# HUBioDataLab/DrugGEN

Measured on AMD Instinct MI355X. Metric: molecules/sec GAN step (G+D fwd+bwd), N=45 graphs, higher is better.
Workload: dtype f32

## Files before the change

druggen_amd/csrc/row_gemm.hip:

```cpp
#include "common.h"
#include "f16_scale.h"
#include "lane_reduce.h"
#include "row_gemm.h"
#include "row_gemm_n384.h"
#include "row_gemm_k384.h"
#include "traversal.h"

#include <cstring>
#include <type_traits>

namespace dg {
namespace {

typedef float f32x16 __attribute__((ext_vector_type(16)));

constexpr int kTR = 64;

struct Epilogue {
    const float* bias = nullptr;
    float* y_alt[2] = {nullptr, nullptr};
    const float* residual = nullptr;
    const float* gamma = nullptr;
    const float* beta = nullptr;
    float* mean = nullptr;
    float* rstd = nullptr;
    float* pre = nullptr;
    float eps = 0.f;
    int relu = 0;
    const float* lnb_pre = nullptr;
    float* lnb_part = nullptr;
    const float* lna_pre = nullptr;
    float* lna_dz = nullptr;
    const float* bias_alt[2] = {nullptr, nullptr};
    int reverse = 0;
};

__device__ __forceinline__ float half_sum(float x) { return half_wave_total_readlane(x, threadIdx.x & 32); }

constexpr int kH3Pitch = 272;
constexpr int kH3Plane = kTR * kH3Pitch;
constexpr int kH3Rs = 2 * kH3Plane;
constexpr int kH3Buf = kH3Rs + kTR * 4;
constexpr int kH3Lds = 2 * kH3Buf;
static_assert(kH3Rs >= kTR * 128 * 4, "the fp32 exchange tile must not reach the row scales");


template <int PFN, int STRIDE>
__device__ __forceinline__ void split_write_h3(const float4 (&set)[PFN], char* pl, int pt) {
    constexpr int G = PFN > 8 ? 2 : 4;
    static_assert(PFN % G == 0 && STRIDE % 32 == 0, "whole groups, whole rows");
    char* const prow = pl + (pt >> 5) * kH3Pitch + (pt & 31) * 8;
    char* const prs = pl + kH3Rs + (pt >> 5) * 4;
#pragma unroll
    for (int g0 = 0; g0 < PFN; g0 += G) {
        unsigned m[G];
#pragma unroll
        for (int j = 0; j < G; ++j) {
            const float4& v = set[g0 + j];
            float t, u;
            asm("v_max3_f32 %0, |%1|, |%2|, |%3|" : "=v"(t) : "v"(v.x), "v"(v.y), "v"(v.z));
            asm("v_max_f32_e64 %0, |%1|, %2" : "=v"(u) : "v"(v.w), "v"(t));
            m[j] = __float_as_uint(u);
        }
#pragma unroll
        for (int j = 0; j < G; ++j) m[j] = umax_dpp<0xB1>(m[j]);
#pragma unroll
        for (int j = 0; j < G; ++j) m[j] = umax_dpp<0x4E>(m[j]);
#pragma unroll
        for (int j = 0; j < G; ++j) m[j] = umax_dpp<0x141>(m[j]);
#pragma unroll
        for (int j = 0; j < G; ++j) m[j] = umax_dpp<0x140>(m[j]);
        float sc[G];
#pragma unroll
        for (int j = 0; j < G; ++j) {
            const auto r = __builtin_amdgcn_permlane16_swap(m[j], m[j], false, false);
            const unsigned x = r[0] > r[1] ? r[0] : r[1];
            const unsigned e = max(x >> 23, 15u);
            m[j] = e;
            sc[j] = scale_of(e);
        }
        f32x2 xa[G], xb[G];
        f16x2 ha[G], hb[G];
#pragma unroll
        for (int j = 0; j < G; ++j) {
            const float4& v = set[g0 + j];
            xa[j] = f32x2{v.x, v.y} * sc[j];
            xb[j] = f32x2{v.z, v.w} * sc[j];
        }
#pragma unroll
        for (int j = 0; j < G; ++j) {
            ha[j] = __builtin_convertvector(xa[j], f16x2);
            hb[j] = __builtin_convertvector(xb[j], f16x2);
        }
#pragma unroll
        for (int j = 0; j < G; ++j) {
            xa[j] -= __builtin_convertvector(ha[j], f32x2);
            xb[j] -= __builtin_convertvector(hb[j], f32x2);
        }
#pragma unroll
        for (int j = 0; j < G; ++j) {
            const f16x2 la = __builtin_convertvector(xa[j], f16x2), lb = __builtin_convertvector(xb[j], f16x2);
            const u32x2 h = {__builtin_bit_cast(unsigned, ha[j]), __builtin_bit_cast(unsigned, hb[j])};
            const u32x2 l = {__builtin_bit_cast(unsigned, la), __builtin_bit_cast(unsigned, lb)};
            *reinterpret_cast<u32x2*>(prow + 0 * kH3Plane + (STRIDE / 32) * (g0 + j) * kH3Pitch) = h;
            *reinterpret_cast<u32x2*>(prow + 1 * kH3Plane + (STRIDE / 32) * (g0 + j) * kH3Pitch) = l;
        }
        if ((pt & 31) == 0) {
#pragma unroll
            for (int j = 0; j < G; ++j)
                *reinterpret_cast<float*>(prs + (STRIDE / 32) * (g0 + j) * 4) = inv_scale_of(m[j]);
        }
    }
}

__device__ __forceinline__ void pack_weight_h3_block(const float* __restrict__ w, const float* __restrict__ w1,
                                                     const float* __restrict__ w2, f16x8* __restrict__ p, int rows, int cols,
                                                     int mode, int n_tiles, int t, int kcb, int kchunks) {
    __shared__ unsigned part[16][32];
    const int k_steps = 8 * kchunks;
    const int lane = threadIdx.x & 63, ks = threadIdx.x >> 6;
    const int c = lane & 31, n = 32 * t + c;
    const int n_out = mode == 0 ? rows : cols, kdim = mode == 0 ? cols : rows;
    auto at = [&](int k) -> float {
        if (n >= n_out || k >= kdim) return 0.f;
        int r = mode == 0 ? n : k;
        const int c = mode == 0 ? k : n;
        const float* ws = w;
        if (w1) {
            ws = r < 128 ? w : (r < 256 ? w1 : w2);
            r &= 127;
        }
        return ws[static_cast<size_t>(r) * cols + c];
    };
    float v[8];
    unsigned mx = 0;
    for (int kc = 0; kc < kchunks; ++kc)
#pragma unroll
        for (int j = 0; j < 8; ++j) {
            const float x = at(kc * 128 + ks * 16 + 8 * (lane >> 5) + j);
            if (kc == kcb) v[j] = x;
            mx = max(mx, __float_as_uint(x) & 0x7FFFFFFFu);
        }
    part[2 * ks + (lane >> 5)][c] = mx;
    __syncthreads();
#pragma unroll
    for (int i = 0; i < 16; ++i) mx = max(mx, part[i][c]);
    const unsigned e = scale_exponent(__uint_as_float(mx));
    const float sc = scale_of(e);
    f16x8 hi, lo;
#pragma unroll
    for (int j = 0; j < 8; ++j) {
        const float xs = v[j] * sc;
        hi[j] = static_cast<_Float16>(xs);
        lo[j] = static_cast<_Float16>(xs - static_cast<float>(hi[j]));
    }
    const size_t slot = static_cast<size_t>(t) * k_steps + 8 * kcb + ks;
    p[(slot * 2 + 0) * 64 + lane] = hi;
    p[(slot * 2 + 1) * 64 + lane] = lo;
    if (kcb == 0 && ks == 0 && lane < 32)
        reinterpret_cast<float*>(p + static_cast<size_t>(n_tiles) * k_steps * 2 * 64)[n] = inv_scale_of(e);
}
__global__ __launch_bounds__(512) void pack_weight_h3_kernel(const float* __restrict__ w, const float* __restrict__ w1,
                                                             const float* __restrict__ w2, f16x8* __restrict__ p, int rows,
                                                             int cols, int mode, int n_tiles) {
    pack_weight_h3_block(w, w1, w2, p, rows, cols, mode, n_tiles, blockIdx.x, blockIdx.y, gridDim.y);
}
__global__ __launch_bounds__(512) void pack_weight_h3_batch_kernel(const long long* __restrict__ table) {
    const long long* e = table + 7 * static_cast<size_t>(blockIdx.z);
    const float* w = reinterpret_cast<const float*>(e[0]);
    f16x8* p = reinterpret_cast<f16x8*>(e[1]);
    const int rows = static_cast<int>(e[2]), cols = static_cast<int>(e[3]), mode = static_cast<int>(e[4]);
    const int n_out = mode == 0 ? rows : cols, k = mode == 0 ? cols : rows;
    const int nt = (n_out + 31) / 32, kc = (k + 127) / 128;
    if (static_cast<int>(blockIdx.x) >= nt || static_cast<int>(blockIdx.y) >= kc) return;
    pack_weight_h3_block(w, reinterpret_cast<const float*>(e[5]), reinterpret_cast<const float*>(e[6]), p, rows, cols, mode,
                         nt, blockIdx.x, blockIdx.y, kc);
}

template <int NG, bool EXCH, bool LNB = false, bool LNA = false>
__global__ __launch_bounds__(512, 2) void row_gemm_h3_kernel(const float* __restrict__ a, const f16x8* __restrict__ packed,
                                                             float* __restrict__ y, int64_t R, Epilogue ep) {
    constexpr int NC = 4, NM = 8 - NC, PFN = 2048 / (64 * NM);
    constexpr int K = 128, KS = 8;
    static_assert(!LNB || (EXCH && NG == 1), "LayerNorm-backward epilogue: 128 -> 128 exchange kernel");
    static_assert(!LNA || (!EXCH && !LNB && NG == 1), "LayerNorm-backward prologue: plain 128 -> 128 kernel");
    static_assert(NG == 1 || (NG == 3 && !EXCH && !LNB && !LNA), "three outputs: direct epilogue, one column group per Linear");
    constexpr int DEPTH = LNA ? 2 : 3;
    extern __shared__ __attribute__((aligned(16))) char smem_raw[];
    char* lds = smem_raw;
    float* xb = reinterpret_cast<float*>(smem_raw + kH3Lds);
    const int lane = threadIdx.x & 63;
    const int w = __builtin_amdgcn_readfirstlane(threadIdx.x >> 6);
    const int half = lane >> 5, col = lane & 31;
    const int64_t tiles = (R + kTR - 1) / kTR;
    if (static_cast<int64_t>(blockIdx.x) >= tiles) return;
    const int64_t my_tiles = (tiles - blockIdx.x + gridDim.x - 1) / gridDim.x;
    const int64_t nchunks = my_tiles;
    const int rot = static_cast<int>(blockIdx.x % 3);
    const int64_t padded = (nchunks + DEPTH - 1) / DEPTH * DEPTH;
    auto tile_at = [&](int64_t ti) {
        const int64_t t = blockIdx.x + ti * gridDim.x;
        if constexpr (LNB || LNA || NG == 3) return t;
        else return ep.reverse ? tiles - 1 - t : t;
    };

    if (w >= NC) {
        const int pt = threadIdx.x - 64 * NC;
        if constexpr (LNA) {
            constexpr int K_ = 128;
            float4 dyr[2][PFN], prr[PFN];
            float st;
            const float4 gam = ld4(ep.gamma + (pt & 31) * 4);
            float4 dgam = f4(0.f), dbet = f4(0.f);
            const unsigned voff0 = static_cast<unsigned>(pt >> 5) * (K_ * 4) + static_cast<unsigned>(pt & 31) * 16;
            auto offsets = [&](int64_t chunk, int64_t& r0, unsigned& lim) {
                r0 = tile_at(chunk) * kTR;
                const int64_t last = R - 1 - r0;
                lim = last >= kTR - 1 ? 0xFFFFFFFFu
                                      : static_cast<unsigned>(last) * (K_ * 4) + static_cast<unsigned>(pt & 31) * 16;
            };
            auto fetch_dy = [&](auto s_tag, int64_t chunk) {
                constexpr int s = decltype(s_tag)::value;
                if (chunk > nchunks - 1) chunk = nchunks - 1;
                int64_t r0;
                unsigned lim;
                offsets(chunk, r0, lim);
                const char* ba = reinterpret_cast<const char*>(a) + r0 * (K_ * 4);
#pragma unroll
                for (int i = 0; i < PFN; ++i) {
                    unsigned off = voff0 + i * (2 * NM * K_ * 4);
                    off = off < lim ? off : lim;
                    dyr[s][i] = ld4(reinterpret_cast<const float*>(ba + off));
                }
            };
            auto fetch_pre = [&](int64_t chunk) {
                if (chunk > nchunks - 1) chunk = nchunks - 1;
                int64_t r0;
                unsigned lim;
                offsets(chunk, r0, lim);
                const char* bp = reinterpret_cast<const char*>(ep.lna_pre) + r0 * (K_ * 4);
#pragma unroll
                for (int i = 0; i < PFN; ++i) {
                    unsigned off = voff0 + i * (2 * NM * K_ * 4);
                    off = off < lim ? off : lim;
                    prr[i] = ld4(reinterpret_cast<const float*>(bp + off));
                }
                int64_t row = r0 + (pt >> 5) + 8 * (pt & 7);
                if (row > R - 1) row = R - 1;
                st = (pt & 8) ? ep.rstd[row] : ep.mean[row];
            };
            auto write2 = [&](auto s_tag, int64_t chunk) {
                constexpr int s = decltype(s_tag)::value;
                const float live = chunk < nchunks ? 1.f : 0.f;
                const int buf = static_cast<int>(chunk & 1);
                if (chunk > nchunks - 1) chunk = nchunks - 1;
                int64_t r0;
                unsigned lim;
                offsets(chunk, r0, lim);
                char* bz = reinterpret_cast<char*>(ep.lna_dz) + r0 * (K_ * 4);
                const int64_t last = R - 1 - r0;
                const unsigned lastu = static_cast<unsigned>(last < kTR - 1 ? last : kTR - 1);
                unsigned rowt = static_cast<unsigned>(pt) >> 5;
                asm volatile("" : "+v"(rowt));
                const int sti = __float_as_int(st);
#pragma unroll
                for (int i0 = 0; i0 < PFN; i0 += 4) {
                    float4 dzs[4];
#pragma unroll
                    for (int i = i0; i < i0 + 4; ++i) {
                        const int mu0 = __builtin_amdgcn_readlane(sti, i), mu1 = __builtin_amdgcn_readlane(sti, 32 + i);
                        const int rs0 = __builtin_amdgcn_readlane(sti, 8 + i), rs1 = __builtin_amdgcn_readlane(sti, 40 + i);
                        const float mu = __int_as_float(half ? mu1 : mu0), rs = __int_as_float(half ? rs1 : rs0);
                        const float4 v = dyr[s][i];
                        const float4 xh = rs * (prr[i] - f4(mu));
                        const float4 u = v * gam;
                        const float c1 = half_sum((u.x + u.y) + (u.z + u.w)) * (1.0f / 128.0f);
                        const float c2 = half_sum((u.x * xh.x + u.y * xh.y) + (u.z * xh.z + u.w * xh.w)) * (1.0f / 128.0f);
                        const float4 dz = rs * (u - f4(c1) - c2 * xh);
                        const float ok = rowt + 8u * i <= lastu ? live : 0.f;
                        const float4 vm = ok * v;
                        dgam = fma4(vm, xh, dgam);
                        dbet += vm;
                        dzs[i - i0] = dz;
                        unsigned off = voff0 + i * (2 * NM * K_ * 4);
                        off = off < lim ? off : lim;
                        st4(reinterpret_cast<float*>(bz + off), dz);
                    }
                    __builtin_amdgcn_sched_barrier(0);
                    split_write_h3<4, 64 * NM>(dzs, lds + buf * kH3Buf, pt + i0 * (64 * NM));
                    __builtin_amdgcn_sched_barrier(0);
                }
                fetch_pre(chunk + 1);
            };
            constexpr std::integral_constant<int, 0> S0{};
            constexpr std::integral_constant<int, 1> S1{};
            fetch_dy(S0, 0);
            fetch_pre(0);
            fetch_dy(S1, 1);
            write2(S0, 0);
            fetch_dy(S0, 2);
            __syncthreads();
            for (int64_t c = 0; c < padded; c += 2) {
                write2(S1, c + 1);
                fetch_dy(S1, c + 3);
                __syncthreads();
                write2(S0, c + 2);
                fetch_dy(S0, c + 4);
                __syncthreads();
            }
            float* pp = ep.lnb_part + (static_cast<size_t>(blockIdx.x) * 8 + 2 * (w - NC) + half) * 256 + (pt & 31) * 4;
            st4(pp, dgam);
            st4(pp + 128, dbet);
            return;
        }
        float4 pf[3][PFN];
        const unsigned voff0 = static_cast<unsigned>(pt >> 5) * (K * 4) + static_cast<unsigned>(pt & 31) * 16;
        auto fetch = [&](float4 (&set)[PFN], int64_t chunk) {
            if (chunk > nchunks - 1) chunk = nchunks - 1;
            const int64_t r0 = tile_at(chunk) * kTR;
            const char* base = reinterpret_cast<const char*>(a) + r0 * (K * 4);
            const int64_t last = R - 1 - r0;
            const unsigned lim = last >= kTR - 1 ? 0xFFFFFFFFu
                                                 : static_cast<unsigned>(last) * (K * 4) + static_cast<unsigned>(pt & 31) * 16;
#pragma unroll
            for (int i = 0; i < PFN; ++i) {
                unsigned off = voff0 + i * (2 * NM * K * 4);
                off = off < lim ? off : lim;
                set[i] = ld4(reinterpret_cast<const float*>(base + off));
            }
        };
        auto write = [&](const float4 (&set)[PFN], int64_t chunk) {
            split_write_h3<PFN, 64 * NM>(set, lds + (chunk & 1) * kH3Buf, pt);
        };
        auto end_of_iteration = [&](int64_t c) {
            if (EXCH && c < nchunks) {
                __syncthreads();
                __syncthreads();
            }
            __syncthreads();
        };
        fetch(pf[0], 0);
        fetch(pf[1], 1);
        fetch(pf[2], 2);
        write(pf[0], 0);
        fetch(pf[0], 3);
        __syncthreads();
        for (int64_t c = 0; c < padded; c += 3) {
            write(pf[1], c + 1);
            fetch(pf[1], c + 4);
            end_of_iteration(c);
            write(pf[2], c + 2);
            fetch(pf[2], c + 5);
            end_of_iteration(c + 1);
            write(pf[0], c + 3);
            fetch(pf[0], c + 6);
            end_of_iteration(c + 2);
        }
        return;
    }

    f16x8 bset[2][2][4];
    auto slab_of = [&](int g) { return 4 * g + w; };
    auto load_b = [&](f16x8 (&bfr)[2][4], int g, int h) {
        const f16x8* wp = packed + static_cast<size_t>(slab_of(g)) * KS * 2 * 64 + lane;
#pragma unroll
        for (int ks = 0; ks < 4; ++ks)
#pragma unroll
            for (int p = 0; p < 2; ++p) bfr[p][ks] = wp[((4 * h + ks) * 2 + p) * 64];
    };
    const float* inv_cs = reinterpret_cast<const float*>(packed + static_cast<size_t>(4 * NG) * KS * 2 * 64);
    float bias_g[NG], cs_g[NG];
#pragma unroll
    for (int g = 0; g < NG; ++g) {
        const int n = 32 * slab_of(g) + col;
        if (NG == 3) {
            const float* bp = n < 128 ? ep.bias : ep.bias_alt[(n >> 7) - 1];
            bias_g[g] = bp ? bp[n & 127] : 0.f;
        } else {
            bias_g[g] = ep.bias ? ep.bias[n] : 0.f;
        }
        cs_g[g] = inv_cs[n];
    }
    float4 res[8];
    float4 lpre[LNB ? 4 : 1];
    float4 dgam = f4(0.f), dbet = f4(0.f);
    f32x16 acc[2];
    auto unit = [&](int64_t ti, int pos_g) {
        const int g = NG > 1 ? (pos_g + rot) % NG : 0;
        const int64_t chunk = ti;
        const int64_t tix = tile_at(ti);
        const int64_t r0 = tix * kTR;
        if (NG > 1) load_b(bset[1], g, 1);
#pragma unroll
        for (int m = 0; m < 2; ++m)
#pragma unroll
            for (int i = 0; i < 16; ++i) acc[m][i] = 0.f;
        unsigned colv = static_cast<unsigned>(col), halfv = static_cast<unsigned>(half);
        if (EXCH) asm volatile("" : "+v"(colv), "+v"(halfv));
        const unsigned lastr = static_cast<unsigned>(R - 1 - r0 < kTR - 1 ? R - 1 - r0 : kTR - 1);
        auto row_off = [&](int it) {
            unsigned rr = static_cast<unsigned>(w * 16 + it * 2) + halfv;
            rr = rr < lastr ? rr : lastr;
            return rr * 512u + colv * 16u;
        };
        if (EXCH && ep.residual) {
            const char* rbase = reinterpret_cast<const char*>(ep.residual) + r0 * 512;
#pragma unroll
            for (int it = 0; it < 8; ++it) res[it] = ld4(reinterpret_cast<const float*>(rbase + row_off(it)));
        }
        const char* pl = lds + (chunk & 1) * kH3Buf;
        f16x8 af[2][2][2];
        auto frags = [&](int ks, f16x8 (&dst)[2][2]) {
#pragma unroll
            for (int m = 0; m < 2; ++m)
#pragma unroll
                for (int p = 0; p < 2; ++p)
                    dst[m][p] = *reinterpret_cast<const f16x8*>(pl + p * kH3Plane + (32 * m + col) * kH3Pitch +
                                                                (ks * 16 + 8 * half) * 2);
        };
        auto row_scales = [&](float4 (&rs)[4], int m, float cs) {
            const float* rsp = reinterpret_cast<const float*>(pl + kH3Rs);
#pragma unroll
            for (int q = 0; q < 4; ++q) rs[q] = cs * ld4(rsp + 32 * m + 8 * q + 4 * half);
        };
        frags(0, af[0]);
#pragma unroll
        for (int ks = 0; ks < 8; ++ks) {
            if (ks + 1 < 8) frags(ks + 1, af[(ks + 1) & 1]);
            if (NG > 1 && ks == 4) {
                const int un = (pos_g + 1) % NG;
                load_b(bset[0], (un + rot) % NG, 0);
            }
            const f16x8(&f)[2][2] = af[ks & 1];
            const f16x8(&bfr)[2][4] = bset[ks >> 2];
            constexpr int TA[3] = {1, 0, 0}, TB[3] = {0, 1, 0};
#pragma unroll
            for (int t = 0; t < 3; ++t)
#pragma unroll
                for (int m = 0; m < 2; ++m)
                    acc[m] = __builtin_amdgcn_mfma_f32_32x32x16_f16(f[m][TA[t]], bfr[TB[t]][ks & 3], acc[m], 0, 0, 0);
        }
        if (!EXCH) {
            const bool full = r0 + kTR <= R;
            const float bias = bias_g[g];
            float* yb = y;
            if constexpr (NG == 3) {
                if (g > 0) yb = ep.y_alt[g - 1];
            }
#pragma unroll
            for (int m = 0; m < 2; ++m) {
                float out[16];
                float4 rs[4];
                row_scales(rs, m, cs_g[g]);
#pragma unroll
                for (int reg = 0; reg < 16; ++reg) {
                    float v = fmaf(acc[m][reg], comp(rs[reg >> 2], reg & 3), bias);
                    if (ep.relu) v = fmaxf(v, 0.f);
                    out[reg] = v;
                }
                float* xw = xb + w * (32 * 32);
#pragma unroll
                for (int reg = 0; reg < 16; ++reg) xw[((reg & 3) + 8 * (reg >> 2) + 4 * half) * 32 + col] = out[reg];
                __builtin_amdgcn_wave_barrier();
                float4 rowv[4];
#pragma unroll
                for (int i = 0; i < 4; ++i) rowv[i] = ld4(xw + (8 * i + (lane >> 3)) * 32 + 4 * (lane & 7));
                __builtin_amdgcn_wave_barrier();
                float* yr = yb + (r0 + 32 * m + (lane >> 3)) * 128 + 32 * w + 4 * (lane & 7);
                if (full) {
#pragma unroll
                    for (int i = 0; i < 4; ++i) st4(yr + static_cast<size_t>(8 * i) * 128, rowv[i]);
                } else {
#pragma unroll
                    for (int i = 0; i < 4; ++i)
                        if (r0 + 32 * m + 8 * i + (lane >> 3) < R) st4(yr + static_cast<size_t>(8 * i) * 128, rowv[i]);
                }
            }
        }
        if (EXCH) {
            float* ex = reinterpret_cast<float*>(lds + (chunk & 1) * kH3Buf);
            const float bias = bias_g[0];
            float4 rs[2][4];
            row_scales(rs[0], 0, cs_g[0]);
            row_scales(rs[1], 1, cs_g[0]);
            if (LNB) {
                const char* pbase = reinterpret_cast<const char*>(ep.lnb_pre) + r0 * 512;
#pragma unroll
                for (int it = 0; it < 4; ++it) lpre[LNB ? it : 0] = ld4(reinterpret_cast<const float*>(pbase + row_off(it)));
            }
            __syncthreads();
#pragma unroll
            for (int m = 0; m < 2; ++m)
#pragma unroll
                for (int reg = 0; reg < 16; ++reg) {
                    const int rr = 32 * m + (reg & 3) + 8 * (reg >> 2) + 4 * half;
                    float v = fmaf(acc[m][reg], comp(rs[m][reg >> 2], reg & 3), bias);
                    if (ep.relu) v = fmaxf(v, 0.f);
                    ex[rr * 128 + 32 * w + col] = v;
                }
            __syncthreads();
            auto finish_rows_lnb = [&](auto check_tag) {
                constexpr bool CHECK = decltype(check_tag)::value;
                float* yrow = reinterpret_cast<float*>(reinterpret_cast<char*>(y + r0 * 128) + ((w * 16 + halfv) * 512u + colv * 16u));
                const float4 gam = ld4(reinterpret_cast<const float*>(reinterpret_cast<const char*>(ep.gamma) + colv * 16u));
#pragma unroll
                for (int hg = 0; hg < 2; ++hg) {
                    float4 pn[4];
                    if (hg == 0) {
                        const char* pbase = reinterpret_cast<const char*>(ep.lnb_pre) + r0 * 512;
#pragma unroll
                        for (int j = 0; j < 4; ++j) pn[j] = ld4(reinterpret_cast<const float*>(pbase + row_off(4 + j)));
                    }
                    float mu4[4], rs4[4];
#pragma unroll
                    for (int j = 0; j < 4; ++j) {
                        unsigned rr = static_cast<unsigned>(w * 16 + (4 * hg + j) * 2) + halfv;
                        rr = rr < lastr ? rr : lastr;
                        mu4[j] = ep.mean[r0 + rr];
                        rs4[j] = ep.rstd[r0 + rr];
                    }
                    float4 yv[4];
#pragma unroll
                    for (int j = 0; j < 4; ++j) {
                        const int it = 4 * hg + j, rr = w * 16 + it * 2 + half;
                        float4 v = ld4(reinterpret_cast<const float*>(reinterpret_cast<const char*>(ex) + ((w * 16 + it * 2 + halfv) * 512u + colv * 16u)));
                        if (ep.residual) v += res[it];
                        if (CHECK && static_cast<unsigned>(w * 16 + it * 2) + halfv > lastr) v = f4(0.f);
                        const float4 xh = rs4[j] * (lpre[LNB ? j : 0] - f4(mu4[j]));
                        const float4 u = v * gam;
                        const float c1 = half_sum((u.x + u.y) + (u.z + u.w)) * (1.0f / 128.0f);
                        const float c2 = half_sum((u.x * xh.x + u.y * xh.y) + (u.z * xh.z + u.w * xh.w)) * (1.0f / 128.0f);
                        yv[j] = rs4[j] * (u - f4(c1) - c2 * xh);
                        dgam = fma4(v, xh, dgam);
                        dbet += v;
                    }
#pragma unroll
                    for (int j = 0; j < 4; ++j) {
                        const int it = 4 * hg + j, rr = w * 16 + it * 2 + half;
                        if (!CHECK || static_cast<unsigned>(w * 16 + it * 2) + halfv <= lastr) st4(yrow + it * 256, yv[j]);
                        if (hg == 0) lpre[LNB ? j : 0] = pn[j];
                    }
                }
            };
            auto finish_rows = [&](auto check_tag) {
                constexpr bool CHECK = decltype(check_tag)::value;
                float* yrow = y + (r0 + w * 16 + half) * 128 + col * 4;
                float* prow = ep.pre ? ep.pre + (r0 + w * 16 + half) * 128 + col * 4 : nullptr;
                float4 gam = f4(0.f), bet = f4(0.f);
                if (ep.gamma) {
                    gam = ld4(ep.gamma + col * 4);
                    bet = ld4(ep.beta + col * 4);
                }
                float4 yv[8], pv[8];
                float mu8[8], rs8[8];
#pragma unroll
                for (int it = 0; it < 8; ++it) {
                    const int rr = w * 16 + it * 2 + half;
                    float4 v = ld4(ex + rr * 128 + col * 4);
                    if (ep.residual) v += res[it];
                    pv[it] = v;
                    if (ep.gamma) {
                        const float mu = half_sum((v.x + v.y) + (v.z + v.w)) * (1.0f / 128.0f);
                        const float4 d = v - f4(mu);
                        const float var = half_sum((d.x * d.x + d.y * d.y) + (d.z * d.z + d.w * d.w)) * (1.0f / 128.0f);
                        const float rs = rsqrtf(var + ep.eps);
                        v = fma4(rs * d, gam, bet);
                        mu8[it] = mu;
                        rs8[it] = rs;
                    }
                    yv[it] = v;
                }
#pragma unroll
                for (int it = 0; it < 8; ++it) {
                    const int rr = w * 16 + it * 2 + half;
                    if (!CHECK || r0 + rr < R) {
                        st4(yrow + it * 256, yv[it]);
                        if (prow && ep.gamma) st4(prow + it * 256, pv[it]);
                    }
                }
                if (ep.gamma && col == 0) {
#pragma unroll
                    for (int it = 0; it < 8; ++it) {
                        const int rr = w * 16 + it * 2 + half;
                        if (!CHECK || r0 + rr < R) {
                            ep.mean[r0 + rr] = mu8[it];
                            ep.rstd[r0 + rr] = rs8[it];
                        }
                    }
                }
            };
            if constexpr (LNB) {
                if (r0 + kTR <= R) finish_rows_lnb(std::false_type{});
                else finish_rows_lnb(std::true_type{});
            } else {
                if (r0 + kTR <= R) finish_rows(std::false_type{});
                else finish_rows(std::true_type{});
            }
        }
        if (pos_g == NG - 1) __syncthreads();
    };
    load_b(bset[0], NG > 1 ? rot : 0, 0);
    if (NG == 1) load_b(bset[1], 0, 1);
    __syncthreads();
    for (int64_t ti = 0; ti < my_tiles; ++ti) {
        if constexpr (NG == 1) {
            unit(ti, 0);
        } else {
#pragma unroll 1
            for (int u = 0; u < NG; ++u) unit(ti, u);
        }
    }
    for (int64_t c = nchunks; c < padded; ++c) __syncthreads();
    if (LNB) {
        float* pp = ep.lnb_part + (static_cast<size_t>(blockIdx.x) * 8 + 2 * w + half) * 256 + col * 4;
        st4(pp, dgam);
        st4(pp + 128, dbet);
    }
}


__device__ __forceinline__ void load_b128_async(f16x8& dst, const f16x8* p) {
    asm volatile("global_load_dwordx4 %0, %1, off" : "=v"(dst) : "v"(p) : "memory");
}
template <int N>
__device__ __forceinline__ void wait_b_refill(f16x8& b0, f16x8& b1) {
    asm volatile("s_waitcnt vmcnt(%2)" : "+v"(b0), "+v"(b1) : "n"(N));
}

struct Sum3Operands {
    const float* a[3];
    const float* residual;
};

template <bool RES>
__global__ __launch_bounds__(512, 2) void row_gemm_h3_sum3_kernel(Sum3Operands in, const f16x8* __restrict__ packed,
                                                                  float* __restrict__ y, int64_t R) {
    constexpr int KC = 3, KS = 24;
    extern __shared__ __attribute__((aligned(16))) char smem_raw[];
    char* lds = smem_raw;
    float* ex = reinterpret_cast<float*>(smem_raw + 2 * kH3Buf);
    const int lane = threadIdx.x & 63;
    const int w = __builtin_amdgcn_readfirstlane(threadIdx.x >> 6);
    const int half = lane >> 5, col = lane & 31;
    const int64_t tiles = (R + kTR - 1) / kTR;
    if (static_cast<int64_t>(blockIdx.x) >= tiles) return;
    const int ntl = static_cast<int>((tiles - blockIdx.x + gridDim.x - 1) / gridDim.x);
    const int npairs = ntl / 2, nchunks = 3 * ntl;
    const int rot = static_cast<int>(blockIdx.x % 3);
    auto tile_row0 = [&](int ti) { return (blockIdx.x + static_cast<int64_t>(ti) * gridDim.x) * kTR; };
    auto chunk_map = [&](int c, int& ti, int& pos) {
        if (c < 6 * npairs) {
            const int p = c / 6, r = c - 6 * p;
            pos = r >> 1;
            ti = 2 * p + (r & 1);
        } else {
            pos = c - 6 * npairs;
            ti = ntl - 1;
        }
    };

    if (w >= 4) {
        __builtin_amdgcn_s_setprio(3);
        const int pw = w - 4, pt = threadIdx.x - 256;
        float4 pf[3][8];
        const unsigned voff0 = static_cast<unsigned>(pt >> 5) * 512 + static_cast<unsigned>(pt & 31) * 16;
        auto fetch = [&](float4 (&set)[8], int c) {
            if (c > nchunks - 1) c = nchunks - 1;
            int ti, pos;
            chunk_map(c, ti, pos);
            const int64_t r0 = tile_row0(ti);
            const int kc = (pos + rot) % KC;
            const char* base = reinterpret_cast<const char*>(in.a[kc]) + r0 * 512;
            const int64_t last = R - 1 - r0;
            const unsigned lim = last >= kTR - 1 ? 0xFFFFFFFFu : static_cast<unsigned>(last) * 512 + static_cast<unsigned>(pt & 31) * 16;
#pragma unroll
            for (int i = 0; i < 8; ++i) {
                unsigned off = voff0 + i * (8 * 512);
                off = off < lim ? off : lim;
                set[i] = ld4(reinterpret_cast<const float*>(base + off));
            }
        };
        auto write = [&](const float4 (&set)[8], int c) {
            split_write_h3<8, 256>(set, lds + (c & 1) * kH3Buf, pt);
        };
        float4 res[8];
        auto fetch_residual = [&](int ti) {
            if (!RES) return;
            const int64_t r0 = tile_row0(ti);
            const char* base = reinterpret_cast<const char*>(in.residual) + r0 * 512;
            const int64_t last = R - 1 - r0;
            const unsigned lim = last >= kTR - 1 ? 0xFFFFFFFFu : static_cast<unsigned>(last) * 512 + col * 16;
            const unsigned roff0 = static_cast<unsigned>(pw * 16 + half) * 512 + col * 16;
#pragma unroll
            for (int it = 0; it < 8; ++it) {
                unsigned off = roff0 + it * 1024;
                off = off < lim ? off : lim;
                res[it] = ld4(reinterpret_cast<const float*>(base + off));
            }
        };
        auto store_tile = [&](int ti) {
            const int64_t r0 = tile_row0(ti);
            const bool full = r0 + kTR <= R;
            float* yrow = y + (r0 + pw * 16 + half) * 128 + col * 4;
#pragma unroll
            for (int hg = 0; hg < 2; ++hg) {
                float4 yv[4];
#pragma unroll
                for (int j = 0; j < 4; ++j) {
                    const int it = 4 * hg + j, rr = pw * 16 + it * 2 + half;
                    yv[j] = ld4(ex + rr * 128 + col * 4);
                    if (RES) yv[j] += res[it];
                }
                if (full) {
#pragma unroll
                    for (int j = 0; j < 4; ++j) st4(yrow + (4 * hg + j) * 256, yv[j]);
                } else {
#pragma unroll
                    for (int j = 0; j < 4; ++j) {
                        const int it = 4 * hg + j, rr = pw * 16 + it * 2 + half;
                        if (r0 + rr < R) st4(yrow + it * 256, yv[j]);
                    }
                }
            }
        };
        fetch(pf[0], 0);
        fetch(pf[1], 1);
        fetch(pf[2], 2);
        write(pf[0], 0);
        fetch(pf[0], 3);
        __syncthreads();
        int c = 0;
        for (int p = 0; p < npairs; ++p, c += 6) {
            const int t0 = 2 * p, t1 = 2 * p + 1;
            write(pf[1], c + 1); fetch(pf[1], c + 4); __syncthreads();
            write(pf[2], c + 2); fetch(pf[2], c + 5); __syncthreads();
            write(pf[0], c + 3); fetch(pf[0], c + 6); __syncthreads();
            write(pf[1], c + 4); fetch(pf[1], c + 7); fetch_residual(t0); __syncthreads();
            write(pf[2], c + 5); fetch(pf[2], c + 8); __syncthreads(); __syncthreads();
            store_tile(t0);
            fetch_residual(t1);
            write(pf[0], c + 6); fetch(pf[0], c + 9); __syncthreads(); __syncthreads();
            store_tile(t1);
        }
        if (ntl & 1) {
            const int t = ntl - 1;
            write(pf[1], c + 1); fetch(pf[1], c + 4); __syncthreads();
            write(pf[2], c + 2); fetch(pf[2], c + 5); fetch_residual(t); __syncthreads();
            write(pf[0], c + 3); __syncthreads(); __syncthreads();
            store_tile(t);
        }
        return;
    }

    f16x8 bfr[2][8];
    auto b_ptr = [&](int pos) { return packed + (static_cast<size_t>(w) * KS + ((pos + rot) % KC) * 8) * 2 * 64 + lane; };
    {
        const f16x8* b0 = b_ptr(0);
#pragma unroll
        for (int ks = 0; ks < 8; ++ks)
#pragma unroll
            for (int p = 0; p < 2; ++p) bfr[p][ks] = b0[(ks * 2 + p) * 64];
    }
    const float cs = reinterpret_cast<const float*>(packed + static_cast<size_t>(4) * KS * 2 * 64)[32 * w + col];
    f32x16 accs[2][2];
    int chunk = 0;
    __syncthreads();
    auto body = [&](int pos, f32x16 (&acc)[2], auto second_tag) {
        constexpr bool SECOND = decltype(second_tag)::value;
        if (pos == 0) {
#pragma unroll
            for (int m = 0; m < 2; ++m)
#pragma unroll
                for (int i = 0; i < 16; ++i) acc[m][i] = 0.f;
        }
        const f16x8* bnext = b_ptr((pos + 1) % KC);
        const char* pl = lds + (chunk & 1) * kH3Buf;
        f16x8 af[2][2][2];
        auto frags = [&](int ks, f16x8 (&dst)[2][2]) {
#pragma unroll
            for (int m = 0; m < 2; ++m)
#pragma unroll
                for (int p = 0; p < 2; ++p)
                    dst[m][p] = *reinterpret_cast<const f16x8*>(pl + p * kH3Plane + (32 * m + col) * kH3Pitch +
                                                                (ks * 16 + 8 * half) * 2);
        };
        f32x16 part[2];
        frags(0, af[0]);
#pragma unroll
        for (int ks = 0; ks < 8; ++ks) {
            if (ks + 1 < 8) frags(ks + 1, af[(ks + 1) & 1]);
            if (!SECOND) {
                switch (ks) {
                    case 0: wait_b_refill<14>(bfr[0][ks], bfr[1][ks]); break;
                    case 1: wait_b_refill<12>(bfr[0][ks], bfr[1][ks]); break;
                    case 2: wait_b_refill<10>(bfr[0][ks], bfr[1][ks]); break;
                    case 3: wait_b_refill<8>(bfr[0][ks], bfr[1][ks]); break;
                    case 4: wait_b_refill<6>(bfr[0][ks], bfr[1][ks]); break;
                    case 5: wait_b_refill<4>(bfr[0][ks], bfr[1][ks]); break;
                    case 6: wait_b_refill<2>(bfr[0][ks], bfr[1][ks]); break;
                    default: wait_b_refill<0>(bfr[0][ks], bfr[1][ks]); break;
                }
            }
            const f16x8(&f)[2][2] = af[ks & 1];
            constexpr int TA[3] = {1, 0, 0}, TB[3] = {0, 1, 0};
#pragma unroll
            for (int t = 0; t < 3; ++t)
#pragma unroll
                for (int m = 0; m < 2; ++m) {
                    if (ks == 0 && t == 0) {
                        const f32x16 zero = {0.f, 0.f, 0.f, 0.f, 0.f, 0.f, 0.f, 0.f, 0.f, 0.f, 0.f, 0.f, 0.f, 0.f, 0.f, 0.f};
                        part[m] = __builtin_amdgcn_mfma_f32_32x32x16_f16(f[m][TA[t]], bfr[TB[t]][ks], zero, 0, 0, 0);
                    } else {
                        part[m] = __builtin_amdgcn_mfma_f32_32x32x16_f16(f[m][TA[t]], bfr[TB[t]][ks], part[m], 0, 0, 0);
                    }
                }
            if (SECOND) {
#pragma unroll
                for (int p = 0; p < 2; ++p) load_b128_async(bfr[p][ks], bnext + (ks * 2 + p) * 64);
            }
        }
        {
            const float* rsp = reinterpret_cast<const float*>(pl + kH3Rs);
#pragma unroll
            for (int m = 0; m < 2; ++m)
#pragma unroll
                for (int q = 0; q < 4; ++q) {
                    const float4 r4 = cs * ld4(rsp + 32 * m + 8 * q + 4 * half);
#pragma unroll
                    for (int i = 0; i < 4; ++i) acc[m][4 * q + i] = fmaf(part[m][4 * q + i], comp(r4, i), acc[m][4 * q + i]);
                }
        }
        if (pos == KC - 1) {
            __syncthreads();
#pragma unroll
            for (int m = 0; m < 2; ++m)
#pragma unroll
                for (int reg = 0; reg < 16; ++reg) {
                    const int rr = 32 * m + (reg & 3) + 8 * (reg >> 2) + 4 * half;
                    ex[rr * 128 + 32 * w + col] = acc[m][reg];
                }
        }
        __syncthreads();
        ++chunk;
    };
    for (int p = 0; p < npairs; ++p) {
#pragma unroll 1
        for (int pos = 0; pos < KC; ++pos) {
            body(pos, accs[0], std::false_type{});
            body(pos, accs[1], std::true_type{});
        }
    }
    if (ntl & 1) {
#pragma unroll 1
        for (int pos = 0; pos < KC; ++pos) {
            body(pos, accs[0], std::false_type{});
            if (pos + 1 < KC) {
                const f16x8* bnext = b_ptr(pos + 1);
#pragma unroll
                for (int ks = 0; ks < 8; ++ks)
#pragma unroll
                    for (int q = 0; q < 2; ++q) load_b128_async(bfr[q][ks], bnext + (ks * 2 + q) * 64);
            }
        }
    }
}

}
}

namespace dg {

size_t row_gemm_f32_packed_floats(int n_out, int k_contract) {
    if (n_out < 1 || k_contract < 1) return 0;
    const size_t nt = (n_out + 31) / 32, kc = (k_contract + 127) / 128;
    return nt * kc * 8 * 2 * 64 * 4 + nt * 32;
}

int row_gemm_f32_pack(const float* w, float* packed, int rows, int cols, int mode, dg_stream_t stream_,
                      const float* w1, const float* w2) {
    if (!w || !packed) return fail(DG_E_ARG, "dg_row_gemm_pack: null pointer");
    if ((w1 || w2) && (!w1 || !w2 || rows != 384))
        return fail(DG_E_ARG, "dg_row_gemm_pack3: needs three [128, cols] weights");
    if (mode != 0 && mode != 1) return fail(DG_E_ARG, "dg_row_gemm_pack: mode must be 0 (forward) or 1 (dgrad)");
    const int n_out = mode == 0 ? rows : cols, k = mode == 0 ? cols : rows;
    const int nt = (n_out + 31) / 32, kc = (k + 127) / 128;
    hipLaunchKernelGGL(pack_weight_h3_kernel, dim3(nt, kc), dim3(512), 0, static_cast<hipStream_t>(stream_), w, w1, w2,
                       reinterpret_cast<f16x8*>(packed), rows, cols, mode, nt);
    return check_launch("dg_row_gemm_pack");
}

int row_gemm_f32_pack_batch(const void* table, int n, int max_rows_cols, dg_stream_t stream_) {
    if (!table) return fail(DG_E_ARG, "dg_row_gemm_pack_batch: null pointer");
    if (n < 1) return 0;
    const int nt = (max_rows_cols + 31) / 32, kc = (max_rows_cols + 127) / 128;
    hipLaunchKernelGGL(pack_weight_h3_batch_kernel, dim3(nt, kc, n), dim3(512), 0, static_cast<hipStream_t>(stream_),
                       static_cast<const long long*>(table));
    return check_launch("dg_row_gemm_pack_batch");
}

size_t row_gemm_f32_mask_words(int64_t R, int K, int N) {
    if (K == 128 && N == 384) return static_cast<size_t>((R + 31) / 32) * 12 * 64;
    if (K == 128 && N == 128) return static_cast<size_t>((R + 63) / 64) * 8 * 64;
    return 0;
}

int row_gemm_f32(const float* a, const float* packed, float* y, int64_t R, int K, int N, const float* bias,
                           int relu, unsigned* relu_bits_out, const unsigned* mask_bits, const float* residual,
                           const float* gamma, const float* beta, float* mean, float* rstd, float* pre_ln,
                           float eps, dg_stream_t stream_, const float* ascale, float* yscale, int afmt, int yfmt,
                           const void* alo, void* ylo) {
    if (!a || !packed || !y) return fail(DG_E_ARG, "dg_row_gemm: null pointer");
    if ((afmt && K != 384) || (yfmt && N != 384)) return fail(DG_E_ARG, "dg_row_gemm: narrow hidden operands are the 384-wide ones");
    if (R < 0 || !((K == 128 && (N == 128 || N == 384)) || (K == 384 && N == 128)))
        return fail(DG_E_SHAPE, "dg_row_gemm: unsupported K=%d N=%d (supported: 128x128, 128x384, 384x128)", K, N);
    if (gamma && (N != 128 || !beta || !mean || !rstd))
        return fail(DG_E_ARG, "dg_row_gemm: LayerNorm epilogue needs N == 128, beta, mean and rstd");
    const bool exch = gamma || residual;
    if (exch && (mask_bits || relu_bits_out))
        return fail(DG_E_ARG, "dg_row_gemm: bit masks cannot be combined with residual / LayerNorm epilogues");
    if ((mask_bits || relu_bits_out) && K != 128)
        return fail(DG_E_ARG, "dg_row_gemm: bit masks need K == 128");
    if (exch && N != 128) return fail(DG_E_ARG, "dg_row_gemm: residual / LayerNorm epilogues need N == 128");
    if ((mask_bits || relu_bits_out) && N != 384)
        return fail(DG_E_ARG, "dg_row_gemm: bit masks need the 128 -> 384 shape");
    if (R == 0) return 0;
    hipStream_t stream = static_cast<hipStream_t>(stream_);
    Epilogue ep;
    ep.bias = bias;
    ep.residual = residual;
    ep.gamma = gamma;
    ep.beta = beta;
    ep.mean = mean;
    ep.rstd = rstd;
    ep.pre = pre_ln;
    ep.eps = eps;
    ep.relu = relu;
    ProfScope prof(R < edge_rows() ? DG_K_ROW_GEMM : (K == 384 ? DG_K_ROW_GEMM_E_K384 : (N == 384 ? DG_K_ROW_GEMM_E_N384 : DG_K_ROW_GEMM_E_128)), stream);
    if (K == 128 && N == 384) {
        if (int st = launch_row_gemm_n384(a, packed, y, yscale, R, bias, relu, relu_bits_out, mask_bits, stream, yfmt, ylo)) return st;
        return check_launch("dg_row_gemm");
    }
    if (K == 384) {
        if (int st = launch_row_gemm_k384(a, ascale, packed, y, R, bias, relu, residual, gamma, beta, mean, rstd, pre_ln, eps, stream, afmt, alo))
            return st;
        return check_launch("dg_row_gemm");
    }
    const int64_t tiles = (R + kTR - 1) / kTR;
    const int seqs = static_cast<int>(tiles < 256 ? tiles : 256);
    ep.reverse = take_direction(R);
#define LAUNCH_H3(EX_)                                                                                         \
    {                                                                                                          \
        constexpr int lds_ = kH3Lds + (EX_ ? 0 : 4 * 32 * 32 * 4);                                            \
        DG_OPT_IN_LDS((&row_gemm_h3_kernel<1, EX_>), lds_);                                                    \
        hipLaunchKernelGGL((row_gemm_h3_kernel<1, EX_>), dim3(seqs), dim3(512), lds_, stream, a,               \
                           reinterpret_cast<const f16x8*>(packed), y, R, ep);                                  \
    }
    if (exch) LAUNCH_H3(true)
    else LAUNCH_H3(false)
#undef LAUNCH_H3
    return check_launch("dg_row_gemm");
}


size_t row_gemm_f32_ln_bwd_workspace_bytes() { return static_cast<size_t>(256) * 8 * 256 * sizeof(float); }

int row_gemm_f32_ln_bwd(const float* a, const float* packed, float* dz, int64_t R, int K, const float* residual,
                        const float* pre, const float* mean, const float* rstd, const float* gamma, float* dgamma,
                        float* dbeta, void* workspace, size_t workspace_bytes, dg_stream_t stream_) {
    if (!a || !packed || !dz || !pre || !mean || !rstd || !gamma || !workspace)
        return fail(DG_E_ARG, "dg_row_gemm_ln_bwd: null pointer");
    if (R < 0 || K != 128) return fail(DG_E_SHAPE, "dg_row_gemm_ln_bwd: unsupported K=%d (K = N = 128)", K);
    if (workspace_bytes < row_gemm_f32_ln_bwd_workspace_bytes()) return fail(DG_E_WORKSPACE, "dg_row_gemm_ln_bwd: workspace too small");
    if (R == 0) return 0;
    hipStream_t stream = static_cast<hipStream_t>(stream_);
    Epilogue ep;
    ep.residual = residual;
    ep.gamma = gamma;
    ep.mean = const_cast<float*>(mean);
    ep.rstd = const_cast<float*>(rstd);
    ep.lnb_pre = pre;
    ep.lnb_part = static_cast<float*>(workspace);
    const int64_t tiles = (R + kTR - 1) / kTR;
    const int seqs = static_cast<int>(tiles < 256 ? tiles : 256);
    {
        ProfScope prof(R < edge_rows() ? DG_K_ROW_GEMM : DG_K_ROW_GEMM_E_128, stream);
        note_forward(R);
        DG_OPT_IN_LDS((&row_gemm_h3_kernel<1, true, true>), kH3Lds);
        hipLaunchKernelGGL((row_gemm_h3_kernel<1, true, true>), dim3(seqs), dim3(512), kH3Lds, stream, a,
                           reinterpret_cast<const f16x8*>(packed), dz, R, ep);
    }
    if (dgamma || dbeta) launch_ln_finish(ep.lnb_part, seqs * 8, 2, 128, dgamma, dbeta, stream);
    return check_launch("dg_row_gemm_ln_bwd");
}

int row_gemm_f32_ln_in(const float* dy, const float* pre, const float* mean, const float* rstd, const float* gamma,
                       const float* packed, float* dz, float* y, float* dgamma, float* dbeta, void* workspace,
                       size_t workspace_bytes, int64_t R, dg_stream_t stream_) {
    if (!dy || !pre || !mean || !rstd || !gamma || !packed || !dz || !y || !workspace)
        return fail(DG_E_ARG, "dg_row_gemm_ln_bwd_in: null pointer");
    if (R < 0) return fail(DG_E_SHAPE, "dg_row_gemm_ln_bwd_in: R = %lld", static_cast<long long>(R));
    if (workspace_bytes < row_gemm_f32_ln_bwd_workspace_bytes()) return fail(DG_E_WORKSPACE, "dg_row_gemm_ln_bwd_in: workspace too small");
    if (R == 0) return 0;
    hipStream_t stream = static_cast<hipStream_t>(stream_);
    Epilogue ep;
    ep.gamma = gamma;
    ep.mean = const_cast<float*>(mean);
    ep.rstd = const_cast<float*>(rstd);
    ep.lna_pre = pre;
    ep.lna_dz = dz;
    ep.lnb_part = static_cast<float*>(workspace);
    const int64_t tiles = (R + kTR - 1) / kTR;
    const int seqs = static_cast<int>(tiles < 256 ? tiles : 256);
    {
        ProfScope prof(R < edge_rows() ? DG_K_ROW_GEMM : DG_K_ROW_GEMM_E_128, stream);
        note_forward(R);
        constexpr int lds = kH3Lds + 4 * 32 * 32 * 4;
        DG_OPT_IN_LDS((&row_gemm_h3_kernel<1, false, false, true>), lds);
        hipLaunchKernelGGL((row_gemm_h3_kernel<1, false, false, true>), dim3(seqs), dim3(512), lds, stream, dy,
                           reinterpret_cast<const f16x8*>(packed), y, R, ep);
    }
    if ((dgamma || dbeta) && !(dgamma && dbeta == dgamma + 128 && reduce_batch_try_add(ep.lnb_part, seqs * 8, 256, dgamma)))
        launch_ln_finish(ep.lnb_part, seqs * 8, 2, 128, dgamma, dbeta, stream);
    return check_launch("dg_row_gemm_ln_bwd_in");
}


int row_gemm_f32_lin3(const float* a, const float* packed, float* y0, float* y1, float* y2, int64_t R, const float* b0,
                      const float* b1, const float* b2, dg_stream_t stream_) {
    if (!a || !packed || !y0 || !y1 || !y2) return fail(DG_E_ARG, "dg_row_gemm_lin3: null pointer");
    if (R < 0) return fail(DG_E_SHAPE, "dg_row_gemm_lin3: negative row count");
    if (R == 0) return 0;
    hipStream_t stream = static_cast<hipStream_t>(stream_);
    Epilogue ep;
    ep.bias = b0;
    ep.y_alt[0] = y1;
    ep.y_alt[1] = y2;
    ep.bias_alt[0] = b1;
    ep.bias_alt[1] = b2;
    const int64_t tiles = (R + kTR - 1) / kTR;
    const int seqs = static_cast<int>(tiles < 256 ? tiles : 256);
    ProfScope prof(R < edge_rows() ? DG_K_ROW_GEMM : DG_K_ROW_GEMM_E_N384, stream);
    constexpr int lds3 = kH3Lds + 4 * 32 * 32 * 4;
    DG_OPT_IN_LDS((&row_gemm_h3_kernel<3, false>), lds3);
    hipLaunchKernelGGL((row_gemm_h3_kernel<3, false>), dim3(seqs), dim3(512), lds3, stream, a,
                       reinterpret_cast<const f16x8*>(packed), y0, R, ep);
    return check_launch("dg_row_gemm_lin3");
}

int row_gemm_f32_sum3(const float* a0, const float* a1, const float* a2, const float* packed, float* y, int64_t R,
                      const float* residual, dg_stream_t stream_) {
    if (!a0 || !a1 || !a2 || !packed || !y) return fail(DG_E_ARG, "dg_row_gemm_sum3: null pointer");
    if (R < 0) return fail(DG_E_SHAPE, "dg_row_gemm_sum3: negative row count");
    if (R == 0) return 0;
    hipStream_t stream = static_cast<hipStream_t>(stream_);
    const Sum3Operands in{{a0, a1, a2}, residual};
    const int64_t tiles = (R + kTR - 1) / kTR;
    const int seqs = static_cast<int>(tiles < 256 ? tiles : 256);
    ProfScope prof(R < edge_rows() ? DG_K_ROW_GEMM : DG_K_ROW_GEMM_E_K384, stream);
    constexpr int lds384 = 2 * kH3Buf + kTR * 128 * 4;
    if (residual) {
        DG_OPT_IN_LDS((&row_gemm_h3_sum3_kernel<true>), lds384);
        hipLaunchKernelGGL((row_gemm_h3_sum3_kernel<true>), dim3(seqs), dim3(512), lds384, stream, in,
                           reinterpret_cast<const f16x8*>(packed), y, R);
    } else {
        DG_OPT_IN_LDS((&row_gemm_h3_sum3_kernel<false>), lds384);
        hipLaunchKernelGGL((row_gemm_h3_sum3_kernel<false>), dim3(seqs), dim3(512), lds384, stream, in,
                           reinterpret_cast<const f16x8*>(packed), y, R);
    }
    return check_launch("dg_row_gemm_sum3");
}

}
```

Measured before the change: 5008.

## Stage residual, LN pre-activations and row stats through LDS in producer warps

In the exchange and LN-backward variants of the h3 row GEMM, the producer wavefronts now prefetch the residual tile, the LN pre-activation tile and the per-row mean/rstd one chunk ahead, then write them into new LDS regions. The consumer epilogue reads those from LDS instead of issuing scattered global loads after the MFMA loop, aiming to take global latency off the epilogue's critical path. Gamma and beta loads are hoisted out of the per-tile loop and pinned in registers. The change raises LDS per workgroup, which could lower occupancy, and adds debug macros (H3_DBG) that are off by default.

```diff
diff --git a/druggen_amd/csrc/row_gemm.hip b/druggen_amd/csrc/row_gemm.hip
--- a/druggen_amd/csrc/row_gemm.hip
+++ b/druggen_amd/csrc/row_gemm.hip
@@ -43,6 +43,15 @@
 constexpr int kH3Buf = kH3Rs + kTR * 4;
 constexpr int kH3Lds = 2 * kH3Buf;
 static_assert(kH3Rs >= kTR * 128 * 4, "the fp32 exchange tile must not reach the row scales");
+constexpr int kH3StRes = kH3Lds;
+constexpr int kH3StPre = kH3StRes + kTR * 512;
+constexpr int kH3StStat = kH3StPre + kTR * 512;
+constexpr int kH3LdsExch = kH3StPre, kH3LdsLnb = kH3StStat + 2 * kTR * 4;
+static_assert(kH3LdsLnb <= 160 * 1024, "one workgroup's LDS");
+
+#ifndef H3_DBG
+#define H3_DBG 0
+#endif
 
 
 template <int PFN, int STRIDE>
@@ -339,19 +348,70 @@
             }
             __syncthreads();
         };
+        float4 sres[EXCH ? PFN : 1], spre[LNB ? PFN : 1];
+        float sst = 0.f;
+        auto stage_fetch = [&](int64_t chunk) {
+            if constexpr (EXCH) {
+                if (chunk > nchunks - 1) chunk = nchunks - 1;
+                const int64_t r0 = tile_at(chunk) * kTR;
+                const int64_t last = R - 1 - r0;
+                const unsigned lim = last >= kTR - 1 ? 0xFFFFFFFFu
+                                                     : static_cast<unsigned>(last) * 512u + static_cast<unsigned>(pt & 31) * 16;
+                const char* rb = ep.residual ? reinterpret_cast<const char*>(ep.residual) + r0 * 512 : reinterpret_cast<const char*>(a);
+                const unsigned rmask = ep.residual ? 0xFFFFFFFFu : 0u;
+                const char* pb = reinterpret_cast<const char*>(ep.lnb_pre) + r0 * 512;
+#pragma unroll
+                for (int i = 0; i < PFN; ++i) {
+                    unsigned off = voff0 + i * (2 * NM * 512);
+                    off = off < lim ? off : lim;
+                    if constexpr (H3_DBG & 4) {
+                        sres[i] = f4(0.f);
+                        if constexpr (LNB) spre[i] = f4(0.f);
+                    } else {
+                        sres[i] = ld4(reinterpret_cast<const float*>(rb + (off & rmask)));
+                        if constexpr (LNB) spre[i] = ld4(reinterpret_cast<const float*>(pb + off));
+                    }
+                }
+                if constexpr (LNB) {
+                    const unsigned lastu = static_cast<unsigned>(last < kTR - 1 ? last : kTR - 1);
+                    unsigned rr = static_cast<unsigned>(pt) & 63u;
+                    rr = rr < lastu ? rr : lastu;
+                    if constexpr (H3_DBG & 4) sst = 1.f;
+                    else sst = ((pt & 64) ? ep.rstd : ep.mean)[r0 + rr];
+                }
+            }
+        };
+        auto stage_write = [&]() {
+            if constexpr (EXCH) {
+                char* d = smem_raw + kH3StRes + (pt >> 5) * 512 + (pt & 31) * 16;
+#pragma unroll
+                for (int i = 0; i < PFN; ++i) {
+                    *reinterpret_cast<float4*>(d + i * (2 * NM * 512)) = sres[i];
+                    if constexpr (LNB) *reinterpret_cast<float4*>(d + (kH3StPre - kH3StRes) + i * (2 * NM * 512)) = spre[i];
+                }
+                if constexpr (LNB) *reinterpret_cast<float*>(smem_raw + kH3StStat + (pt & 127) * 4) = sst;
+            }
+        };
         fetch(pf[0], 0);
         fetch(pf[1], 1);
         fetch(pf[2], 2);
+        stage_fetch(0);
         write(pf[0], 0);
         fetch(pf[0], 3);
         __syncthreads();
         for (int64_t c = 0; c < padded; c += 3) {
+            stage_write();
+            stage_fetch(c + 1);
             write(pf[1], c + 1);
             fetch(pf[1], c + 4);
             end_of_iteration(c);
+            stage_write();
+            stage_fetch(c + 2);
             write(pf[2], c + 2);
             fetch(pf[2], c + 5);
             end_of_iteration(c + 1);
+            stage_write();
+            stage_fetch(c + 3);
             write(pf[0], c + 3);
             fetch(pf[0], c + 6);
             end_of_iteration(c + 2);
@@ -381,8 +441,12 @@
         }
         cs_g[g] = inv_cs[n];
     }
+    const char* const st_res = smem_raw + kH3StRes;
+    const char* const st_pre = smem_raw + kH3StPre;
+    const float* const st_stat = reinterpret_cast<const float*>(smem_raw + kH3StStat);
     float4 res[8];
     float4 lpre[LNB ? 4 : 1];
+    float4 gam = f4(0.f), bet = f4(0.f);
     float4 dgam = f4(0.f), dbet = f4(0.f);
     f32x16 acc[2];
     auto unit = [&](int64_t ti, int pos_g) {
@@ -397,17 +461,13 @@
             for (int i = 0; i < 16; ++i) acc[m][i] = 0.f;
         unsigned colv = static_cast<unsigned>(col), halfv = static_cast<unsigned>(half);
         if (EXCH) asm volatile("" : "+v"(colv), "+v"(halfv));
+        if (LNB) asm volatile("" : "+v"(dbet.x), "+v"(dbet.y), "+v"(dbet.z), "+v"(dbet.w));
         const unsigned lastr = static_cast<unsigned>(R - 1 - r0 < kTR - 1 ? R - 1 - r0 : kTR - 1);
         auto row_off = [&](int it) {
             unsigned rr = static_cast<unsigned>(w * 16 + it * 2) + halfv;
             rr = rr < lastr ? rr : lastr;
             return rr * 512u + colv * 16u;
         };
-        if (EXCH && ep.residual) {
-            const char* rbase = reinterpret_cast<const char*>(ep.residual) + r0 * 512;
-#pragma unroll
-            for (int it = 0; it < 8; ++it) res[it] = ld4(reinterpret_cast<const float*>(rbase + row_off(it)));
-        }
         const char* pl = lds + (chunk & 1) * kH3Buf;
         f16x8 af[2][2][2];
         auto frags = [&](int ks, f16x8 (&dst)[2][2]) {
@@ -438,7 +498,8 @@
             for (int t = 0; t < 3; ++t)
 #pragma unroll
                 for (int m = 0; m < 2; ++m)
-                    acc[m] = __builtin_amdgcn_mfma_f32_32x32x16_f16(f[m][TA[t]], bfr[TB[t]][ks & 3], acc[m], 0, 0, 0);
+                    if constexpr (!(EXCH && (H3_DBG & 1)))
+                        acc[m] = __builtin_amdgcn_mfma_f32_32x32x16_f16(f[m][TA[t]], bfr[TB[t]][ks & 3], acc[m], 0, 0, 0);
         }
         if (!EXCH) {
             const bool full = r0 + kTR <= R;
@@ -483,11 +544,6 @@
             float4 rs[2][4];
             row_scales(rs[0], 0, cs_g[0]);
             row_scales(rs[1], 1, cs_g[0]);
-            if (LNB) {
-                const char* pbase = reinterpret_cast<const char*>(ep.lnb_pre) + r0 * 512;
-#pragma unroll
-                for (int it = 0; it < 4; ++it) lpre[LNB ? it : 0] = ld4(reinterpret_cast<const float*>(pbase + row_off(it)));
-            }
             __syncthreads();
 #pragma unroll
             for (int m = 0; m < 2; ++m)
@@ -499,25 +555,31 @@
                     ex[rr * 128 + 32 * w + col] = v;
                 }
             __syncthreads();
+            if (ep.residual) {
+#pragma unroll
+                for (int it = 0; it < 8; ++it) res[it] = ld4(reinterpret_cast<const float*>(st_res + row_off(it)));
+            }
+            if (LNB) {
+#pragma unroll
+                for (int it = 0; it < 4; ++it) lpre[LNB ? it : 0] = ld4(reinterpret_cast<const float*>(st_pre + row_off(it)));
+            }
             auto finish_rows_lnb = [&](auto check_tag) {
                 constexpr bool CHECK = decltype(check_tag)::value;
                 float* yrow = reinterpret_cast<float*>(reinterpret_cast<char*>(y + r0 * 128) + ((w * 16 + halfv) * 512u + colv * 16u));
-                const float4 gam = ld4(reinterpret_cast<const float*>(reinterpret_cast<const char*>(ep.gamma) + colv * 16u));
 #pragma unroll
                 for (int hg = 0; hg < 2; ++hg) {
                     float4 pn[4];
                     if (hg == 0) {
-                        const char* pbase = reinterpret_cast<const char*>(ep.lnb_pre) + r0 * 512;
-#pragma unroll
-                        for (int j = 0; j < 4; ++j) pn[j] = ld4(reinterpret_cast<const float*>(pbase + row_off(4 + j)));
+#pragma unroll
+                        for (int j = 0; j < 4; ++j) pn[j] = ld4(reinterpret_cast<const float*>(st_pre + row_off(4 + j)));
                     }
                     float mu4[4], rs4[4];
 #pragma unroll
                     for (int j = 0; j < 4; ++j) {
                         unsigned rr = static_cast<unsigned>(w * 16 + (4 * hg + j) * 2) + halfv;
                         rr = rr < lastr ? rr : lastr;
-                        mu4[j] = ep.mean[r0 + rr];
-                        rs4[j] = ep.rstd[r0 + rr];
+                        mu4[j] = st_stat[rr];
+                        rs4[j] = st_stat[kTR + rr];
                     }
                     float4 yv[4];
 #pragma unroll
@@ -537,7 +599,8 @@
 #pragma unroll
                     for (int j = 0; j < 4; ++j) {
                         const int it = 4 * hg + j, rr = w * 16 + it * 2 + half;
-                        if (!CHECK || static_cast<unsigned>(w * 16 + it * 2) + halfv <= lastr) st4(yrow + it * 256, yv[j]);
+                        if constexpr (H3_DBG & 2) dbet += yv[j];
+                        else if (!CHECK || static_cast<unsigned>(w * 16 + it * 2) + halfv <= lastr) st4(yrow + it * 256, yv[j]);
                         if (hg == 0) lpre[LNB ? j : 0] = pn[j];
                     }
                 }
@@ -546,11 +609,6 @@
                 constexpr bool CHECK = decltype(check_tag)::value;
                 float* yrow = y + (r0 + w * 16 + half) * 128 + col * 4;
                 float* prow = ep.pre ? ep.pre + (r0 + w * 16 + half) * 128 + col * 4 : nullptr;
-                float4 gam = f4(0.f), bet = f4(0.f);
-                if (ep.gamma) {
-                    gam = ld4(ep.gamma + col * 4);
-                    bet = ld4(ep.beta + col * 4);
-                }
                 float4 yv[8], pv[8];
                 float mu8[8], rs8[8];
 #pragma unroll
@@ -601,6 +659,17 @@
     };
     load_b(bset[0], NG > 1 ? rot : 0, 0);
     if (NG == 1) load_b(bset[1], 0, 1);
+    if constexpr (EXCH) {
+        if (LNB || ep.gamma) gam = ld4(ep.gamma + col * 4);
+        if (!LNB && ep.gamma) bet = ld4(ep.beta + col * 4);
+#pragma unroll
+        for (int h = 0; h < 2; ++h)
+#pragma unroll
+            for (int p = 0; p < 2; ++p)
+                asm volatile("" ::"v"(bset[h][p][0]), "v"(bset[h][p][1]), "v"(bset[h][p][2]), "v"(bset[h][p][3]));
+        asm volatile("" ::"v"(gam.x), "v"(gam.y), "v"(gam.z), "v"(gam.w), "v"(bet.x), "v"(bet.y), "v"(bet.z), "v"(bet.w),
+                     "v"(bias_g[0]), "v"(cs_g[0]));
+    }
     __syncthreads();
     for (int64_t ti = 0; ti < my_tiles; ++ti) {
         if constexpr (NG == 1) {
@@ -950,7 +1019,7 @@
     ep.reverse = take_direction(R);
 #define LAUNCH_H3(EX_)                                                                                         \
     {                                                                                                          \
-        constexpr int lds_ = kH3Lds + (EX_ ? 0 : 4 * 32 * 32 * 4);                                            \
+        constexpr int lds_ = EX_ ? kH3LdsExch : kH3Lds + 4 * 32 * 32 * 4;                                     \
         DG_OPT_IN_LDS((&row_gemm_h3_kernel<1, EX_>), lds_);                                                    \
         hipLaunchKernelGGL((row_gemm_h3_kernel<1, EX_>), dim3(seqs), dim3(512), lds_, stream, a,               \
                            reinterpret_cast<const f16x8*>(packed), y, R, ep);                                  \
@@ -985,8 +1054,8 @@
     {
         ProfScope prof(R < edge_rows() ? DG_K_ROW_GEMM : DG_K_ROW_GEMM_E_128, stream);
         note_forward(R);
-        DG_OPT_IN_LDS((&row_gemm_h3_kernel<1, true, true>), kH3Lds);
-        hipLaunchKernelGGL((row_gemm_h3_kernel<1, true, true>), dim3(seqs), dim3(512), kH3Lds, stream, a,
+        DG_OPT_IN_LDS((&row_gemm_h3_kernel<1, true, true>), kH3LdsLnb);
+        hipLaunchKernelGGL((row_gemm_h3_kernel<1, true, true>), dim3(seqs), dim3(512), kH3LdsLnb, stream, a,
                            reinterpret_cast<const f16x8*>(packed), dz, R, ep);
     }
     if (dgamma || dbeta) launch_ln_finish(ep.lnb_part, seqs * 8, 2, 128, dgamma, dbeta, stream);
```

New measurement: 4990. About the same (-0.4%).
